# troubling/hummingbird

Hardware: AMD Instinct MI355X
Metric: GiB/s device-resident EC encode+reconstruct, 4+2 @ 1 MiB; % HBM roofline (higher is better)
Workload: dtype u8; 1 GPU; 4+2 Encode + Reconstruct{0,1} of 4096 x 1 MiB objects per GPU, device-resident (BASELINE configs[1]+[2]); k=4, m=2, object_bytes=1048576, objects_per_gpu=4096, global_objects=4096, parallelism=object-partition x1

## Files before the change

hummingbird_amd/csrc/hbec.cpp:

```cpp
#include <hip/hip_runtime.h>

#include <algorithm>
#include <atomic>
#include <condition_variable>
#include <cstdio>
#include <cstdlib>
#include <cstring>
#include <deque>
#include <map>
#include <memory>
#include <mutex>
#include <string>
#include <vector>

#include "../../include/hbec.h"
#include "gf256.h"
#include "internal.h"
#include "kernels.h"
#include "mixed.h"

namespace hbec {

static thread_local std::string t_last_error;

int fail(int code, const std::string& msg) {
    t_last_error = msg;
    return code;
}

int hip_fail(hipError_t e, const char* what) {
    (void)hipGetLastError();
    std::string m = std::string(what) + ": " + hipGetErrorString(e);
    return fail(e == hipErrorOutOfMemory ? HBEC_ERR_NOMEM : HBEC_ERR_DEVICE, m);
}

long long hbec::env_knob(const char* name, long long dflt) {
    const char* e = std::getenv(name);
    return e && *e ? std::atoll(e) : dflt;
}

static std::atomic<int> g_force_stream{0};
static const int g_unaligned_bpc = (int)tune_knob("HBEC_UNALIGNED_BPC", 0);
static const int g_blocks_per_cu_override = (int)tune_knob("HBEC_BLOCKS_PER_CU", 0);
static const int g_grid_cap_env = (int)tune_knob("HBEC_GRID_CAP", 0);
thread_local int t_grid_cap = 0;
void set_thread_grid_cap(int blocks) { t_grid_cap = blocks; }
#define g_grid_cap (t_grid_cap > 0 ? (g_grid_cap_env > 0 ? std::min(t_grid_cap, g_grid_cap_env) : t_grid_cap) : g_grid_cap_env)
static const uint64_t g_chunk_tiles = [] {
    const long long v = tune_knob("HBEC_CHUNK_TILES", 0);
    return (uint64_t)(v > 0 ? v : (1ll << 20));
}();
static std::atomic<uint64_t> g_odd_chunk_override{0};
static uint64_t odd_chunk_tiles() {
    const uint64_t v = g_odd_chunk_override.load(std::memory_order_relaxed);
    return v ? v : g_chunk_tiles;
}
static const uint64_t g_vec_chunk_tiles = [] {
    const long long v = tune_knob("HBEC_VEC_CHUNK_TILES", tune_knob("HBEC_CHUNK_TILES", 0));
    return (uint64_t)(v > 0 ? v : HBEC_VEC_CHUNK_TILES);
}();

struct DeviceInfo {
    int cus = 0;
    std::map<std::pair<int, int>, int> blocks_per_cu;
};

static std::mutex g_dev_mu;
static std::map<int, DeviceInfo> g_devs;

static int bpc_occ_cap(int k, int r) {
    int b = 1;
    if (verify_occupancy(k, r, &b) != hipSuccess) return 1;
    return b;
}

static int current_device(int* dev) {
    hipError_t e = hipGetDevice(dev);
    if (e != hipSuccess) return hip_fail(e, "hipGetDevice");
    return HBEC_OK;
}

static int device_blocks(int dev, int k, int r, int pipe, int force_stream, int* cus, int* per_cu) {
    std::lock_guard<std::mutex> g(g_dev_mu);
    DeviceInfo& d = g_devs[dev];
    if (d.cus == 0) {
        hipDeviceProp_t p;
        hipError_t e = hipGetDeviceProperties(&p, dev);
        if (e != hipSuccess) return hip_fail(e, "hipGetDeviceProperties");
        d.cus = p.multiProcessorCount;
    }
    const int key_k = pipe == 3 ? 3000 : (force_stream ? -k : (pipe == 2 ? 2000 + k : (pipe ? 1000 + k : k)));
    auto it = d.blocks_per_cu.find({key_k, r});
    if (it == d.blocks_per_cu.end()) {
        int b = 0;
        hipError_t e = pipe == 3   ? unaligned_occupancy(r, &b)
                       : pipe == 2 ? packed_occupancy(k, r, &b)
                                   : vec_occupancy(k, r, pipe, force_stream, &b);
        if (e != hipSuccess) return hip_fail(e, "occupancy query");
        if (b < 1) b = 1;
        it = d.blocks_per_cu.emplace(std::make_pair(key_k, r), b).first;
    }
    *cus = d.cus;
    *per_cu = it->second;
    return HBEC_OK;
}

static int cu_count(int dev, int* cus) {
    std::lock_guard<std::mutex> g(g_dev_mu);
    DeviceInfo& d = g_devs[dev];
    if (d.cus == 0) {
        hipDeviceProp_t p;
        hipError_t e = hipGetDeviceProperties(&p, dev);
        if (e != hipSuccess) return hip_fail(e, "hipGetDeviceProperties");
// ... 211 lines not shown
        return apply_wide(rows, cols, coeffs, in, out, n_obj, shard_len, stream);

    for (int r0 = 0; r0 < rows; r0 += kMaxR) {
        const int R = std::min(kMaxR, rows - r0);
        for (int c0 = 0; c0 < cols; c0 += kMaxK) {
            const int K = std::min(kMaxK, cols - c0);
            PassArgs a;
            std::memset(&a, 0, sizeof(a));
            for (int j = 0; j < K; ++j) {
                a.in[j] = static_cast<const uint8_t*>(in[c0 + j].base);
                a.in_stride[j] = in[c0 + j].obj_stride;
            }
            for (int r = 0; r < R; ++r) {
                a.out[r] = static_cast<uint8_t*>(out[r0 + r].base);
                a.out_stride[r] = out[r0 + r].obj_stride;
                for (int j = 0; j < K; ++j) perm_table(coeffs[(size_t)(r0 + r) * cols + c0 + j], a.tab[r][j]);
            }
            a.shard_len = shard_len;
            a.accumulate = c0 > 0 ? 1u : 0u;
            if (vec && is_packed_shape(K, R, shard_len, c0 > 0, force_stream)) {
                int cus = 0, per_cu = 0;
                rc = device_blocks(dev, K, R, 2, 0, &cus, &per_cu);
                if (rc) return rc;
                const uint64_t spo = shard_len / 16;
                const uint64_t te = (uint64_t)packed_tile_elems(K);
                uint64_t max_obj = std::max<uint64_t>(1, ((1ull << 31) - te) / spo);
                max_obj = std::min(max_obj, std::max<uint64_t>(1, g_chunk_tiles * te / spo));
                for (uint64_t o0 = 0; o0 < n_obj; o0 += max_obj) {
                    const uint64_t no = std::min(max_obj, n_obj - o0);
                    PassArgs b = a;
                    for (int j = 0; j < K; ++j) b.in[j] = a.in[j] + o0 * a.in_stride[j];
                    for (int r = 0; r < R; ++r) b.out[r] = a.out[r] + o0 * a.out_stride[r];
                    b.n_obj = no;
                    b.elems_per_obj = (uint32_t)spo;
                    b.n_elems = (uint32_t)(no * spo);
                    b.n_tiles = (uint32_t)((no * spo + te - 1) / te);
                    const uint64_t wpb = (uint64_t)kPipeBlockThreads / 64;
                    const uint64_t want_blocks = (b.n_tiles + wpb - 1) / wpb;
                    const uint64_t cap = (uint64_t)cus * (uint64_t)(g_blocks_per_cu_override > 0
                                                                         ? g_blocks_per_cu_override
                                                                         : per_cu);
                    int grid = (int)std::max<uint64_t>(1, std::min(want_blocks, cap));
                    if (g_grid_cap > 0) grid = std::min(grid, g_grid_cap);
                    hipError_t e = launch_packed(K, R, b, grid, stream);
                    if (e != hipSuccess) return hip_fail(e, "launch gf_apply_packed");
                }
            } else if (vec && !to_rec) {
                int cus = 0, per_cu = 0;
                rc = device_blocks(dev, K, R, is_pipe_shape(K, R, shard_len, force_stream) && c0 == 0, force_stream,
                                   &cus, &per_cu);
                if (rc) return rc;
                const uint64_t tile = (uint64_t)vec_tile_bytes(K, R, shard_len, c0 > 0, force_stream);
                const uint64_t tpo = (shard_len + tile - 1) / tile;
                const uint64_t max_obj = std::max<uint64_t>(1, std::min<uint64_t>((1ull << 31), g_vec_chunk_tiles) / tpo);
                for (uint64_t o0 = 0; o0 < n_obj; o0 += max_obj) {
                    const uint64_t no = std::min(max_obj, n_obj - o0);
                    PassArgs b = a;
                    for (int j = 0; j < K; ++j) b.in[j] = a.in[j] + o0 * a.in_stride[j];
                    for (int r = 0; r < R; ++r) b.out[r] = a.out[r] + o0 * a.out_stride[r];
                    b.n_obj = no;
                    b.tiles_per_obj = (uint32_t)tpo;
                    b.n_tiles = (uint32_t)(no * tpo);
                    const uint64_t wpb = (uint64_t)vec_block_threads(K, R, shard_len, c0 > 0, force_stream) / 64;
                    const uint64_t want_blocks = (b.n_tiles + wpb - 1) / wpb;
                    const uint64_t cap = (uint64_t)cus * (uint64_t)(g_blocks_per_cu_override > 0
                                                                         ? g_blocks_per_cu_override
                                                                         : per_cu);
                    int grid = (int)std::max<uint64_t>(1, std::min(want_blocks, cap));
                    if (g_grid_cap > 0) grid = std::min(grid, g_grid_cap);
                    hipError_t e = launch_vec(K, R, b, grid, stream, force_stream);
                    if (e != hipSuccess) return hip_fail(e, "launch gf_apply_vec");
                }
            } else if (odd_enabled() && cols <= kOddMaxK && pos32_shard(shard_len)) {
                rc = apply_odd(a, K, R, c0 > 0, n_obj, shard_len, dev, stream);
                if (rc) return rc;
            } else {
                int cus = 0, per_cu = 0;
                rc = device_blocks(dev, K, R, 3, 0, &cus, &per_cu);
                if (rc) return rc;
                if (g_unaligned_bpc > 0) per_cu = std::min(per_cu, g_unaligned_bpc);
                const uint64_t tpo = unaligned_tiles_per_obj(shard_len);
                const uint64_t max_obj = std::max<uint64_t>(1, std::min<uint64_t>((1ull << 31), g_chunk_tiles) / tpo);
                for (uint64_t o0 = 0; o0 < n_obj; o0 += max_obj) {
                    const uint64_t no = std::min(max_obj, n_obj - o0);
                    PassArgs b = a;
                    for (int j = 0; j < K; ++j) b.in[j] = a.in[j] + o0 * a.in_stride[j];
                    for (int r = 0; r < R; ++r) b.out[r] = a.out[r] + o0 * a.out_stride[r];
                    b.n_obj = no;
                    b.tiles_per_obj = (uint32_t)tpo;
                    b.n_tiles = (uint32_t)(no * tpo);
                    const uint64_t want_blocks = (b.n_tiles + kBlockThreads / 64 - 1) / (kBlockThreads / 64);
                    int grid = (int)std::max<uint64_t>(1, std::min<uint64_t>(want_blocks, (uint64_t)cus * per_cu));
                    if (g_grid_cap > 0) grid = std::min(grid, g_grid_cap);
                    hipError_t e = launch_unaligned(K, R, b, grid, stream);
                    if (e != hipSuccess) return hip_fail(e, "launch gf_apply_unaligned");
                }
            }
        }
    }
    return HBEC_OK;
}

struct Staging {
    int dev = 0;
    hipStream_t stream = nullptr;
    uint8_t* dbuf = nullptr;
    size_t dcap = 0;
    uint8_t* hbuf = nullptr;
    uint64_t hbuf_dev = 0;
    size_t hcap = 0;
    std::vector<hipEvent_t> ev;
};

static const bool g_percall_mapped = tune_knob("HBEC_PERCALL_DMA", 0) == 0;

static const int g_percall_pieces = (int)std::max(1LL, std::min(16LL, tune_knob("HBEC_PERCALL_PIECES", 2)));

class PercallGate {
  public:
    explicit PercallGate(int limit) : limit_(limit) {}
    void enter() {
        if (limit_ <= 0) return;
        std::unique_lock<std::mutex> lk(mu_);
        if (running_ < limit_ && waiters_.empty()) {
            ++running_;
// ... 363 lines not shown
    const int k = c->k;
    std::vector<MixedRec> recs;
    uint64_t slice[kMaxR + 2] = {};
    std::vector<uint64_t> first;
    uint64_t n_ent = 0;
    for (int r = 1; r <= kMaxR; ++r) {
        slice[r] = n_ent;
        for (MixedPattern& p : pats) {
            if (!p.uses || (int)p.outs.size() != r) continue;
            MixedRec m;
            std::memset(&m, 0, sizeof(m));
            for (int j = 0; j < k; ++j) {
                m.in_base[j] = reinterpret_cast<uint64_t>(views[p.surv[j]].base);
                m.in_stride[j] = views[p.surv[j]].obj_stride;
            }
            for (int q = 0; q < r; ++q) {
                m.out_base[q] = reinterpret_cast<uint64_t>(views[p.outs[q]].base);
                m.out_stride[q] = views[p.outs[q]].obj_stride;
                for (int j = 0; j < k; ++j) perm_table(p.rows[(size_t)q * k + j], m.tab[q][j]);
            }
            p.rec = (uint32_t)recs.size();
            recs.push_back(m);
            first.push_back(n_ent);
            n_ent += p.uses;
        }
    }
    slice[kMaxR + 1] = n_ent;
    if (n_ent == 0) return HBEC_OK;
    std::vector<MixedEnt> ents((size_t)n_ent);
    for (uint64_t o = 0; o < n_objects; ++o) {
        const MixedPattern& p = pats[pattern_of[o]];
        if (p.outs.empty()) continue;
        ents[(size_t)first[p.rec]++] = MixedEnt{(uint32_t)o, p.rec};
    }

    int dev = 0, cus = 0;
    int rc = current_device(&dev);
    if (rc) return rc;
    rc = cu_count(dev, &cus);
    if (rc) return rc;
    const size_t rec_bytes = recs.size() * sizeof(MixedRec), ent_bytes = ents.size() * sizeof(MixedEnt);
    void* d = nullptr;
    rc = scratch_alloc(rec_bytes + ent_bytes, stream, &d);
    if (rc) return rc;
    const MixedRec* d_recs = static_cast<const MixedRec*>(d);
    const MixedEnt* d_ents = reinterpret_cast<const MixedEnt*>(static_cast<const uint8_t*>(d) + rec_bytes);
    hipError_t e = hipMemcpyAsync(d, recs.data(), rec_bytes, hipMemcpyHostToDevice, stream);
    if (e == hipSuccess)
        e = hipMemcpyAsync(const_cast<MixedEnt*>(d_ents), ents.data(), ent_bytes, hipMemcpyHostToDevice, stream);

    const uint64_t tile = (uint64_t)mixed_tile_bytes(k);
    const uint64_t tpo = (shard_len + tile - 1) / tile;
    const uint64_t hook = g_mixed_chunk_override.load(std::memory_order_relaxed);
    const uint64_t max_ent = std::max<uint64_t>(1, std::min<uint64_t>((1ull << 31) - 1, hook ? hook : g_vec_chunk_tiles) / tpo);
    constexpr uint64_t wpb = kBlockThreads / 64;
    for (int r = 1; r <= kMaxR && e == hipSuccess; ++r) {
        for (uint64_t e0 = slice[r]; e0 < slice[r + 1] && e == hipSuccess; e0 += max_ent) {
            const uint64_t ne = std::min(max_ent, slice[r + 1] - e0);
            MixedArgs a;
            a.n_tiles = (uint32_t)(ne * tpo);
            a.tiles_per_obj = (uint32_t)tpo;
            a.shard_len = (uint32_t)shard_len;
            int grid = (int)std::max<uint64_t>(1, std::min<uint64_t>((a.n_tiles + wpb - 1) / wpb, (uint64_t)cus));
            if (g_grid_cap > 0) grid = std::min(grid, g_grid_cap);
            const uint64_t waves = (uint64_t)grid * wpb;
            a.iters = (uint32_t)((a.n_tiles + waves - 1) / waves);
            const uint64_t n_recs = ents[(size_t)(e0 + ne - 1)].rec - ents[(size_t)e0].rec + 1;
            const bool contig = mixed_contiguous(waves, tpo, ne, n_recs);
            a.wave_step = contig ? a.iters : 1u;
            a.iter_step = contig ? 1u : (uint32_t)waves;
            g_mixed_launches.fetch_add(1, std::memory_order_relaxed);
            e = launch_mixed(k, r, a, d_recs, d_ents + e0, grid, stream);
        }
    }
    scratch_free(d, stream);
    if (e != hipSuccess) return hip_fail(e, "launch gf_apply_mixed");
    return HBEC_OK;
}

static int reconstruct_mixed(hbec_codec* c, const hbec_view* views, const uint8_t* patterns, uint32_t n_patterns,
                             const uint32_t* pattern_of, uint64_t n_objects, uint64_t shard_len, bool data_only,
                             hipStream_t stream) {
    if (!c || !views || !patterns || !pattern_of) return fail(HBEC_ERR_INVALID_ARG, "null argument");
    if (n_patterns > 65536) return fail(HBEC_ERR_INVALID_ARG, "more than 65536 patterns");
    if (n_objects && !n_patterns) return fail(HBEC_ERR_INVALID_ARG, "objects but no patterns");
    const int k = c->k, n = c->k + c->m;
    std::vector<MixedPattern> pats(n_patterns);
    std::vector<std::vector<uint8_t>> masks(n_patterns);
    for (uint32_t p = 0; p < n_patterns; ++p) {
        masks[p].assign(patterns + (size_t)p * n, patterns + (size_t)(p + 1) * n);
        int n_present = 0;
        for (auto& v : masks[p]) n_present += (v = v ? 1 : 0);
        if (n_present < k) return fail(HBEC_ERR_TOO_FEW_SHARDS, "too few shards given (pattern " + std::to_string(p) + ")");
    }
    for (uint64_t o = 0; o < n_objects; ++o) {
        if (pattern_of[o] >= n_patterns)
            return fail(HBEC_ERR_INVALID_ARG, "pattern index out of range (object " + std::to_string(o) + ")");
        ++pats[pattern_of[o]].uses;
    }
    bool fast = k <= kMixedMaxK && shard_len % 16 == 0 && pos32_shard(shard_len) && n_objects < (1ull << 32);
    for (uint32_t p = 0; p < n_patterns; ++p) {
        MixedPattern& mp = pats[p];
        if (!mp.uses) continue;
        int rc = decode_rows(c, masks[p], data_only, mp.surv, mp.outs, mp.rows);
        if (rc) return rc;
        if (mp.outs.empty()) continue;
        fast = fast && (int)mp.outs.size() <= kMaxR;
// ... 614 lines not shown
        return HBEC_OK;
    });
}

int hbec_set_odd_chunk_tiles(uint64_t tiles) {
    g_odd_chunk_override.store(tiles, std::memory_order_relaxed);
    return HBEC_OK;
}

int hbec_set_force_stream(int on) {
    return hbec::guarded("hbec_set_force_stream", [&]() -> int {
        g_force_stream.store(on ? 1 : 0);
        return HBEC_OK;
    });
}

int hbec_kernel_info(int k, int r, uint64_t shard_len, int* tile_bytes, int* kind, int* blocks_per_cu) {
    return hbec::guarded("hbec_kernel_info", [&]() -> int {
        if (k < 1 || k > kMaxK || r < 1 || r > kMaxR) return fail(HBEC_ERR_INVALID_ARG, "shape out of range");
        const int fs = g_force_stream.load();
        const bool packed = r <= 3 && is_packed_shape(k, r, shard_len, 0, fs);
        const bool rec = !packed && shard_len % 16 == 0 && rec_route(k, r, shard_len, shard_len % 128 == 0, false);
        const int pipe = packed ? 2 : is_pipe_shape(k, r, shard_len, fs);
        if (tile_bytes)
            *tile_bytes = packed ? packed_tile_elems(k) * 16
                                 : (rec ? (int)odd_rec_tile_span(k, 0, -1) : vec_tile_bytes(k, r, shard_len, 0, fs));
        if (kind) *kind = packed ? 3 : (rec ? 4 : (is_streaming_shape(k, r, fs) ? 2 : (pipe ? 1 : 0)));
        if (blocks_per_cu) {
            int dev = 0, cus = 0;
            int rc = current_device(&dev);
            if (rc) return rc;
            rc = device_blocks(dev, k, r, pipe, packed ? 0 : fs, &cus, blocks_per_cu);
            if (rc) return rc;
            if (rec) *blocks_per_cu = odd_blocks_per_cu(0, k, r, false, true);
            if (g_blocks_per_cu_override > 0) *blocks_per_cu = g_blocks_per_cu_override;
        }
        return HBEC_OK;
    });
}

}

extern "C" int hbec_odd_record_cache(int clear, uint64_t* entries, uint64_t* hits) {
    return hbec::guarded("hbec_odd_record_cache", [&]() -> int {
        ObjRecCache& C = objrec_cache();
        std::lock_guard<std::mutex> lk(C.mu);
        if (clear) {
            hipError_t e = hipDeviceSynchronize();
            if (e != hipSuccess) return hip_fail(e, "hipDeviceSynchronize (record cache)");
            for (auto& x : C.entries) {
                if (x.ev) (void)hipEventDestroy(x.ev);
                if (x.d) (void)hipFree(x.d);
            }
            C.entries.clear();
            C.seen.clear();
            C.bytes = 0;
            C.hits = 0;
        }
        if (entries) *entries = C.entries.size();
        if (hits) *hits = C.hits;
        return HBEC_OK;
    });
}
```

hummingbird_amd/csrc/kernels.h:

```cpp
#pragma once
#include <hip/hip_runtime.h>
#include <stdint.h>

#include "tuning.h"

namespace hbec {

long long env_knob(const char* name, long long dflt);
inline long long tune_knob(const char* name, long long dflt) {
#if HBEC_TUNE
    return env_knob(name, dflt);
#else
    (void)name;
    return dflt;
#endif
}

constexpr int kMaxK = 16;
constexpr uint32_t kOddListWords = 4;
constexpr int kMaxR = 4;
constexpr int kBlockThreads = 256;
constexpr int kPipeBlockThreads = HBEC_PIPE_BLOCK;
constexpr int kPipeBlocksPerCu = HBEC_PIPE_BLOCKS_PER_CU;

constexpr int kVecWavesPerSimd = HBEC_WAVES_PER_SIMD;

struct PassArgs {
    const uint8_t* in[kMaxK];
    uint64_t in_stride[kMaxK];
    uint8_t* out[kMaxR];
    uint64_t out_stride[kMaxR];
    uint32_t tab[kMaxR][kMaxK][5];
    uint64_t n_obj;
    uint64_t shard_len;
    uint32_t tiles_per_obj;
    uint32_t n_tiles;
    uint32_t accumulate;
    uint32_t n_elems;
    uint32_t elems_per_obj;
    uint32_t fuse;
    const uint32_t* list;
};

int is_packed_shape(int k, int r, uint64_t shard_len, int accumulate, int force_stream);
int packed_tile_elems(int k);
hipError_t launch_packed(int k, int r, const PassArgs& a, int grid, hipStream_t stream);
hipError_t packed_occupancy(int k, int r, int* blocks_per_cu);

int vec_tile_bytes(int k, int r, uint64_t shard_len, int accumulate, int force_stream);
int is_streaming_shape(int k, int r, int force_stream);
int is_pipe_shape(int k, int r, uint64_t shard_len, int force_stream);
int vec_block_threads(int k, int r, uint64_t shard_len, int accumulate, int force_stream);
__host__ __device__ constexpr int pipe_u(int k) { return k <= 4 ? (4 / k) : (k <= 8 ? HBEC_PIPE_U_BIG : 1); }

__host__ __device__ constexpr int stripes_u(int k) { return k <= 4 ? pipe_u(k) : 1; }
__host__ __device__ constexpr int verify_u(int k) { return k <= 4 ? 4 : 1; }

hipError_t launch_vec(int k, int r, const PassArgs& a, int grid, hipStream_t stream, int force_stream);
uint32_t unaligned_tiles_per_obj(uint64_t shard_len);
hipError_t launch_unaligned(int k, int r, const PassArgs& a, int grid, hipStream_t stream);
hipError_t unaligned_occupancy(int r, int* blocks_per_cu);
struct URec {
    uint64_t a;
    uint64_t b;
    uint64_t shard_len;
    uint64_t p0;
};
struct UPlanArgs {
    const URec* recs;
    uint32_t n_recs;
    uint32_t accumulate;
    uint32_t in_idx[kMaxK];
    uint32_t out_idx[kMaxR];
    uint32_t in_sel, out_sel;
    uint32_t tab[kMaxR][kMaxK][5];
    uint32_t mirror;
    uint32_t carry;
};
uint32_t unaligned_tile_bytes();
hipError_t launch_verify_unaligned(int k, int r, const PassArgs& a, uint32_t* flags, int grid, hipStream_t stream);
hipError_t launch_unaligned_plan(int k, int r, const UPlanArgs& a, int grid, hipStream_t stream);
constexpr int kOddMaxK = 12;
constexpr uint64_t kPos32MaxShard = (1ull << 31) - (1ull << 16);
__host__ __device__ constexpr bool pos32_shard(uint64_t shard_len) { return shard_len <= kPos32MaxShard; }
bool odd_enabled();
int odd_blocks_per_cu(int mode, int k, int r, bool mirror = false, bool records = false, int xs = -1);
bool odd_supported(int k, int r);
uint64_t urec_tile();
uint64_t urec_tile_for(int k, bool mirror);
uint64_t urec_span(uint64_t shard_len);
uint32_t odd_tile_bytes(int k);
uint32_t odd_plan_tile_bytes();
uint32_t odd_tiles_per_obj(int k, int mode, uint64_t shard_len, bool records, int xs = -1);
uint64_t odd_frame_tiles(uint64_t shard_len, uint64_t tile);
int odd_bp_schedule(int k, int r, int mode, const uint32_t (*tab)[kMaxK][5], bool plan);
uint32_t odd_rec_tile_span(int k, int mode, int xs);
uint32_t odd_waves_per_block(int xs);
uint64_t odd_min_main();
bool odd_uses_records(int k, int r);
uint32_t odd_rec_words(int k, int r, int mode);
hipError_t launch_odd_objrec(int k, int r, int mode, const PassArgs& a, uint32_t* recs, hipStream_t stream);
hipError_t launch_odd_planrec(int k, int r, int mode, const UPlanArgs& p, const URec* orecs, uint32_t n,
                              uint32_t* recs, hipStream_t stream);
hipError_t launch_odd(int k, int r, int mode, const PassArgs& a, uint32_t* flags, const uint32_t* recs, int grid,
// ... 82 lines not shown
```

hummingbird_amd/csrc/kernels.hip:

```cpp
#include <hip/hip_runtime.h>
#include <stdint.h>

#include <cstdlib>
#include <cstring>

#include "gf_device.h"
#include "kernels.h"

namespace hbec {

template <int K, int R, int U>
__device__ __forceinline__ void process_tile(const PassArgs& a, const Tables<K, R>& tb, uint64_t obj,
                                             uint64_t off0, bool full, bool accumulate) {
    u32x4 x[U][K];
    const uint64_t last = a.shard_len - 16u;
#pragma unroll
    for (int u = 0; u < U; ++u) {
        uint64_t off = off0 + (uint64_t)u * 1024u;
        if (!full) off = off < last ? off : last;
#pragma unroll
        for (int j = 0; j < K; ++j) x[u][j] = ld16(a.in[j] + obj * a.in_stride[j] + off);
    }
    u32x4 old[U][R];
    if (accumulate) {
// ... 105 lines not shown
        load_tile<K, R, U>(nxt, a, obj_n, base_n + lane * 16u);
        if (K <= 4) __builtin_amdgcn_s_sleep(HBEC_PIPE_SLEEP);
        if (base + TILE <= a.shard_len)
            compute_store_tile<K, R, U>(cur, a, tb, obj, base + lane * 16u, true);
        else
            compute_store_tile<K, R, U>(cur, a, tb, obj, base + lane * 16u, false);
#pragma unroll
        for (int u = 0; u < U; ++u)
#pragma unroll
            for (int j = 0; j < K; ++j) cur[u][j] = nxt[u][j];
        obj = obj_n;
        base = base_n;
    }
    if (base + TILE <= a.shard_len)
        compute_store_tile<K, R, U>(cur, a, tb, obj, base + lane * 16u, true);
    else
        compute_store_tile<K, R, U>(cur, a, tb, obj, base + lane * 16u, false);
}

template <int K, int R>
struct PipeTile {
    uint64_t in[K];
    uint64_t out[R];
    uint32_t valid;
    uint32_t live;
};

template <int K, int R, int U>
__device__ __forceinline__ void pipe_tile_coords(PipeTile<K, R>& b, const PassArgs& a, uint32_t t, uint32_t tpo) {
    constexpr uint64_t TILE = (uint64_t)U * 1024u;
    const uint32_t obj = t / tpo;
    const uint64_t off = (uint64_t)(t - obj * tpo) * TILE;
#pragma unroll
    for (int j = 0; j < K; ++j) b.in[j] = reinterpret_cast<uint64_t>(a.in[j]) + obj * a.in_stride[j] + off;
#pragma unroll
    for (int r = 0; r < R; ++r) b.out[r] = reinterpret_cast<uint64_t>(a.out[r]) + obj * a.out_stride[r] + off;
    const uint64_t left = a.shard_len - off;
    b.valid = (uint32_t)(left < TILE ? left : TILE);
    b.live = b.valid;
}

template <int K, int R, int U>
__device__ __forceinline__ void pipe2_load(u32x4 (&x)[U][K], const PipeTile<K, R>& b, uint32_t lane) {
    const uint64_t last = (uint64_t)b.valid - 16u;
#pragma unroll
    for (int q = 0; q < U * K; ++q) {
        const int u = HBEC_PIPE_IMAJ ? q % U : q / K, j = HBEC_PIPE_IMAJ ? q / U : q % K;
        uint64_t off = (uint64_t)lane * 16u + (uint64_t)u * 1024u;
        off = off < last ? off : last;
        x[u][j] = HBEC_PIPE_TEMP ? ld16_addr_t(b.in[j] + off) : ld16_addr(b.in[j] + off);
    }
}

template <int K, int R, int U, bool FULL>
__device__ __forceinline__ void pipe2_store_(const u32x4 (&x)[U][K], const PassArgs& a, const Tables<K, R>& tb,
                                             const PipeTile<K, R>& b, uint32_t lane) {
#pragma unroll
    for (int u = 0; u < U; ++u) {
        const uint64_t off = (uint64_t)lane * 16u + (uint64_t)u * 1024u;
        u32x4 acc[R];
#pragma unroll
        for (int r = 0; r < R; ++r) acc[r] = u32x4{0, 0, 0, 0};
        gf_dot<K, R>(acc, x[u], a.tab, tb);
        if (FULL || off < b.live) {
#pragma unroll
            for (int r = 0; r < R; ++r) st16_addr(b.out[r] + off, acc[r]);
        }
    }
}

template <int K, int R, int U>
__device__ __forceinline__ void pipe_tile_at(PipeTile<K, R>& b, const PassArgs& a, uint32_t t, uint32_t n,
                                             uint32_t tpo) {
    pipe_tile_coords<K, R, U>(b, a, t < n ? t : n - 1u, tpo);
    if (t >= n) b.live = 0;
}

template <int K, int R, int U>
__device__ __forceinline__ void pipe2_finish(const u32x4 (&x)[U][K], const PassArgs& a, const Tables<K, R>& tb,
                                             const PipeTile<K, R>& cur, uint32_t lane) {
    if (cur.live >= (uint32_t)U * 1024u)
        pipe2_store_<K, R, U, true>(x, a, tb, cur, lane);
    else
        pipe2_store_<K, R, U, false>(x, a, tb, cur, lane);
}


template <int K, int R>
__global__ __launch_bounds__(kPipeBlockThreads, 1) void gf_apply_vec_pipe2(PassArgs a) {
    constexpr int U = pipe_u(K);
    constexpr uint32_t WPB = kPipeBlockThreads / 64;
    const uint32_t lane = threadIdx.x & 63u;
    const uint32_t nw = gridDim.x * WPB;
    const uint32_t wave0 = __builtin_amdgcn_readfirstlane(xcd_block() * WPB);
    const uint32_t dw = __builtin_amdgcn_readfirstlane(threadIdx.x >> 6);
    const uint32_t wave = wave0 + dw;
    const uint32_t tpo = a.tiles_per_obj;
    const uint32_t n = a.n_tiles;
    if (wave0 >= n) return;
    const Tables<K, R> tb = load_tables<K, R>(a.tab);
    PipeTile<K, R> cur, nxt;
    pipe_tile_at<K, R, U>(cur, a, wave, n, tpo);
    u32x4 x[U][K];
    pipe2_load<K, R, U>(x, cur, lane);
    pipe_tile_at<K, R, U>(nxt, a, wave + nw, n, tpo);
    for (uint32_t b0 = wave0 + nw; b0 < n; b0 += nw) {
        u32x4 y[U][K];
        pipe2_load<K, R, U>(y, nxt, lane);
        if (K <= 4) __builtin_amdgcn_s_sleep(HBEC_PIPE2_SLEEP);
        __builtin_amdgcn_s_barrier();
        PipeTile<K, R> after;
        pipe_tile_at<K, R, U>(after, a, b0 + dw + nw, n, tpo);
        pipe2_finish<K, R, U>(x, a, tb, cur, lane);
#pragma unroll
        for (int u = 0; u < U; ++u)
#pragma unroll
            for (int j = 0; j < K; ++j) x[u][j] = y[u][j];
        cur = nxt;
        nxt = after;
    }
    pipe2_finish<K, R, U>(x, a, tb, cur, lane);
}

template <int K, int U>
__device__ __forceinline__ void packed_load(u32x4 (&x)[U][K], const PassArgs& a, const PackedCoord<U>& c) {
#pragma unroll
    for (int u = 0; u < U; ++u)
#pragma unroll
        for (int j = 0; j < K; ++j) x[u][j] = ld16(a.in[j] + (uint64_t)c.obj[u] * a.in_stride[j] + c.off[u]);
}

template <int K, int R, int U, bool FULL>
__device__ __forceinline__ void packed_store_(const u32x4 (&x)[U][K], const PassArgs& a, const Tables<K, R>& tb,
                                              const PackedCoord<U>& c, uint32_t t, uint32_t lane, uint32_t live) {
#pragma unroll
    for (int u = 0; u < U; ++u) {
        u32x4 acc[R];
#pragma unroll
        for (int r = 0; r < R; ++r) acc[r] = u32x4{0, 0, 0, 0};
        gf_dot<K, R>(acc, x[u], a.tab, tb);
        if (FULL || (t * (uint32_t)U + (uint32_t)u) * 64u + lane < live) {
#pragma unroll
            for (int r = 0; r < R; ++r) st16(a.out[r] + (uint64_t)c.obj[u] * a.out_stride[r] + c.off[u], acc[r]);
        }
    }
}

template <int K, int R, int U>
__device__ __forceinline__ void packed_finish(const u32x4 (&x)[U][K], const PassArgs& a, const Tables<K, R>& tb,
                                              const PackedCoord<U>& c, uint32_t t, uint32_t n, uint32_t lane) {
    const uint32_t live = t < n ? a.n_elems : 0u;
    if (t < n && (t + 1u) * (uint32_t)U * 64u <= a.n_elems)
        packed_store_<K, R, U, true>(x, a, tb, c, t, lane, live);
    else
        packed_store_<K, R, U, false>(x, a, tb, c, t, lane, live);
}


__host__ __device__ constexpr int packed_u(int k) {
    return k > 4 ? HBEC_PACKED_U_BIG : pipe_u(k);
}

template <int K, int R>
__global__ __launch_bounds__(kPipeBlockThreads, 1) void gf_apply_packed(PassArgs a) {
    constexpr int U = packed_u(K);
    constexpr uint32_t WPB = kPipeBlockThreads / 64;
    const uint32_t lane = threadIdx.x & 63u;
    const uint32_t nw = gridDim.x * WPB;
    const uint32_t wave0 = __builtin_amdgcn_readfirstlane(xcd_block() * WPB);
    const uint32_t dw = __builtin_amdgcn_readfirstlane(threadIdx.x >> 6);
    const uint32_t n = a.n_tiles;
    if (wave0 >= n) return;
    const Tables<K, R> tb = load_tables<K, R>(a.tab);
    const uint32_t spo = a.elems_per_obj;
    const double inv = 1.0 / (double)spo;
// ... 391 lines not shown
static uint64_t packed_max_shard(int k) {
    if (k > 4) return HBEC_PACKED_MAX_BIG;
    const uint64_t tile = (uint64_t)pipe_u(k) * 1024u;
    return tile > 2048u ? tile : 2048u;
}

static const bool g_packed_on = tune_knob("HBEC_PACKED", 1) != 0;
static const uint64_t g_packed_max = (uint64_t)std::max(0LL, tune_knob("HBEC_PACKED_MAX_SHARD", 0));

int is_packed_shape(int k, int r, uint64_t shard_len, int accumulate, int force_stream) {
    return (g_packed_on && !force_stream && !accumulate && shard_len >= 16 && shard_len % 16 == 0 &&
            shard_len < (g_packed_max ? g_packed_max : packed_max_shard(k)) &&
            packed_kernel(k, r) != nullptr)
               ? 1
               : 0;
}

hipError_t launch_packed(int k, int r, const PassArgs& a, int grid, hipStream_t stream) {
    const void* fn = packed_kernel(k, r);
    if (!fn) return hipErrorInvalidValue;
    void* args[] = {const_cast<PassArgs*>(&a)};
    return hipLaunchKernel(fn, dim3(grid), dim3(kPipeBlockThreads), args, 0, stream);
}


hipError_t packed_occupancy(int k, int r, int* blocks_per_cu) {
    const void* fn = packed_kernel(k, r);
    if (!fn) return hipErrorInvalidValue;
    hipError_t e = hipOccupancyMaxActiveBlocksPerMultiprocessor(blocks_per_cu, fn, kPipeBlockThreads, 0);
    const int cap = k <= 4 ? HBEC_PACKED_BLOCKS_SMALL : HBEC_PACKED_BLOCKS_BIG;
    if (e == hipSuccess && cap > 0 && *blocks_per_cu > cap) *blocks_per_cu = cap;
    return e;
}

static bool use_pipe(int k, uint64_t shard_len, bool accumulate) {
    return !accumulate && shard_len >= (uint64_t)pipe_u(k) * 1024u;
}

int is_pipe_shape(int k, int r, uint64_t shard_len, int force_stream) {
    return (!is_streaming_shape(k, r, force_stream) && use_pipe(k, shard_len, false)) ? 1 : 0;
}

int vec_tile_bytes(int k, int r, uint64_t shard_len, int accumulate, int force_stream) {
    if (!force_stream && unrolled_kernel(k, r, false))
        return (use_pipe(k, shard_len, accumulate != 0) ? pipe_u(k) : tile_kib(k)) * 1024;
    return 4 * 1024;
}

int vec_block_threads(int k, int r, uint64_t shard_len, int accumulate, int force_stream) {
    return (!is_streaming_shape(k, r, force_stream) && use_pipe(k, shard_len, accumulate != 0)) ? kPipeBlockThreads
                                                                                               : kBlockThreads;
}

hipError_t launch_vec(int k, int r, const PassArgs& a, int grid, hipStream_t stream, int force_stream) {
    const bool pipe = use_pipe(k, a.shard_len, a.accumulate != 0);
    const void* fn = force_stream ? nullptr : unrolled_kernel(k, r, pipe);
    if (fn) {
        void* args[] = {const_cast<PassArgs*>(&a)};
        return hipLaunchKernel(fn, dim3(grid), dim3(pipe ? kPipeBlockThreads : kBlockThreads), args, 0, stream);
    }
    fn = stream_kernel(r);
    if (!fn || k < 1 || k > kMaxK) return hipErrorInvalidValue;
    void* args[] = {const_cast<PassArgs*>(&a), &k};
    return hipLaunchKernel(fn, dim3(grid), dim3(kBlockThreads), args, 0, stream);
}


static const void* unaligned_kernel(int r) {
    switch (r) {
        case 1: return reinterpret_cast<const void*>(&gf_apply_unaligned<1>);
        case 2: return reinterpret_cast<const void*>(&gf_apply_unaligned<2>);
        case 3: return reinterpret_cast<const void*>(&gf_apply_unaligned<3>);
        case 4: return reinterpret_cast<const void*>(&gf_apply_unaligned<4>);
    }
    return nullptr;
}

uint32_t unaligned_tiles_per_obj(uint64_t shard_len) {
    const uint64_t windows = (shard_len + kUnalignedWindow - 1) / kUnalignedWindow;
    return (uint32_t)((windows + kUnalignedU - 1) / kUnalignedU);
}

hipError_t launch_unaligned(int k, int r, const PassArgs& a, int grid, hipStream_t stream) {
    const void* fn = unaligned_kernel(r);
    if (!fn || k < 1 || k > kMaxK) return hipErrorInvalidValue;
    void* args[] = {const_cast<PassArgs*>(&a), &k};
    return hipLaunchKernel(fn, dim3(grid), dim3(kBlockThreads), args, 0, stream);
}

static const void* unaligned_plan_kernel(int r) {
    switch (r) {
        case 1: return reinterpret_cast<const void*>(&gf_apply_unaligned_plan<1>);
        case 2: return reinterpret_cast<const void*>(&gf_apply_unaligned_plan<2>);
        case 3: return reinterpret_cast<const void*>(&gf_apply_unaligned_plan<3>);
        case 4: return reinterpret_cast<const void*>(&gf_apply_unaligned_plan<4>);
    }
    return nullptr;
}

hipError_t launch_verify_unaligned(int k, int r, const PassArgs& a, uint32_t* flags, int grid, hipStream_t stream) {
    const void* fn = nullptr;
    switch (r) {
        case 1: fn = reinterpret_cast<const void*>(&gf_verify_unaligned<1>); break;
        case 2: fn = reinterpret_cast<const void*>(&gf_verify_unaligned<2>); break;
        case 3: fn = reinterpret_cast<const void*>(&gf_verify_unaligned<3>); break;
        case 4: fn = reinterpret_cast<const void*>(&gf_verify_unaligned<4>); break;
    }
    if (!fn || k < 1 || k > kMaxK) return hipErrorInvalidValue;
    void* args[] = {const_cast<PassArgs*>(&a), &k, &flags};
    return hipLaunchKernel(fn, dim3(grid), dim3(kBlockThreads), args, 0, stream);
}

uint32_t unaligned_tile_bytes() { return (uint32_t)kUnalignedU * kUnalignedWindow; }

hipError_t launch_unaligned_plan(int k, int r, const UPlanArgs& a, int grid, hipStream_t stream) {
    const void* fn = unaligned_plan_kernel(r);
    if (!fn || k < 1 || k > kMaxK) return hipErrorInvalidValue;
    void* args[] = {const_cast<UPlanArgs*>(&a), &k};
    return hipLaunchKernel(fn, dim3(grid), dim3(kBlockThreads), args, 0, stream);
}

hipError_t unaligned_occupancy(int r, int* blocks_per_cu) {
    const void* fn = unaligned_kernel(r);
    if (!fn) return hipErrorInvalidValue;
    return hipOccupancyMaxActiveBlocksPerMultiprocessor(blocks_per_cu, fn, kBlockThreads, 0);
}

hipError_t launch_fill(uint8_t* dst, uint64_t n_obj, uint64_t obj_len, uint64_t obj_stride, uint64_t base_seed,
                       uint64_t first, int grid, hipStream_t stream) {
    hipLaunchKernelGGL(fill_splitmix, dim3(grid), dim3(kBlockThreads), 0, stream, dst, n_obj, obj_len, obj_stride,
                       base_seed, first);
    return hipGetLastError();
}

struct PutWords {
    uint32_t n;
    uint32_t w[kPutWordsMax];
};
__global__ __launch_bounds__(kBlockThreads) void put_words(uint32_t* __restrict__ dst, PutWords a) {
    for (uint32_t i = threadIdx.x; i < a.n; i += blockDim.x) dst[i] = a.w[i];
}

hipError_t launch_put_words(void* dst, const void* src, size_t bytes, hipStream_t stream) {
    if (bytes % 4 != 0) return hipErrorInvalidValue;
    const uint32_t* w = static_cast<const uint32_t*>(src);
    uint32_t* d = static_cast<uint32_t*>(dst);
    for (size_t i = 0, n = bytes / 4; i < n; i += kPutWordsMax) {
        PutWords a;
        a.n = (uint32_t)std::min<size_t>(kPutWordsMax, n - i);
        std::memcpy(a.w, w + i, (size_t)a.n * 4);
        hipLaunchKernelGGL(put_words, dim3(1), dim3(kBlockThreads), 0, stream, d + i, a);
        const hipError_t e = hipGetLastError();
        if (e != hipSuccess) return e;
    }
    return hipSuccess;
}

hipError_t vec_occupancy(int k, int r, int pipe, int force_stream, int* blocks_per_cu) {
    const void* fn = force_stream ? nullptr : unrolled_kernel(k, r, pipe != 0);
    const bool is_pipe = fn && pipe;
    if (!fn) fn = stream_kernel(r);
    if (!fn) return hipErrorInvalidValue;
    hipError_t e = hipOccupancyMaxActiveBlocksPerMultiprocessor(blocks_per_cu, fn,
                                                                is_pipe ? kPipeBlockThreads : kBlockThreads, 0);
    if (e == hipSuccess && is_pipe && kPipeBlocksPerCu > 0 && *blocks_per_cu > kPipeBlocksPerCu)
        *blocks_per_cu = kPipeBlocksPerCu;
    return e;
}

}
```

hummingbird_amd/csrc/tuning.h:

```cpp
#pragma once

#ifndef HBEC_TUNE
#define HBEC_TUNE 0
#endif

#ifndef HBEC_PIPE_BLOCK
#define HBEC_PIPE_BLOCK 256
#endif
#ifndef HBEC_PIPE_BLOCKS_PER_CU
#define HBEC_PIPE_BLOCKS_PER_CU 1
#endif
#ifndef HBEC_PIPE_U_BIG
#define HBEC_PIPE_U_BIG 3
#endif
#ifndef HBEC_PIPE_SLEEP
#define HBEC_PIPE_SLEEP 6
#endif
#ifndef HBEC_PIPE2_SLEEP
#define HBEC_PIPE2_SLEEP 8
#endif
#ifndef HBEC_PIPE_IMAJ
#define HBEC_PIPE_IMAJ 0
#endif
#ifndef HBEC_PIPE_TEMP
#define HBEC_PIPE_TEMP 0
#endif
#ifndef HBEC_VEC_CHUNK_TILES
#define HBEC_VEC_CHUNK_TILES 262144
#endif
#ifndef HBEC_PIPE_V2_MAXK
#define HBEC_PIPE_V2_MAXK 4
#endif

#ifndef HBEC_WAVES_PER_SIMD
#define HBEC_WAVES_PER_SIMD 4
#endif
#ifndef HBEC_TILE_SMALL
#define HBEC_TILE_SMALL 4
#endif
#ifndef HBEC_TILE_MID
#define HBEC_TILE_MID 1
#endif
#ifndef HBEC_TILE_BIG
#define HBEC_TILE_BIG 1
#endif

#ifndef HBEC_ALLVGPR_MIN
#define HBEC_ALLVGPR_MIN 16
#endif

#ifndef HBEC_PACKED_U_BIG
#define HBEC_PACKED_U_BIG 1
#endif
#ifndef HBEC_PACKED_MAX_BIG
#define HBEC_PACKED_MAX_BIG 32784
#endif
#ifndef HBEC_PACKED_BLOCKS_SMALL
#define HBEC_PACKED_BLOCKS_SMALL 2
#endif
#ifndef HBEC_PACKED_BLOCKS_BIG
#define HBEC_PACKED_BLOCKS_BIG 1
#endif
#ifndef HBEC_VERIFY_PACKED_U_SMALL
#define HBEC_VERIFY_PACKED_U_SMALL 2
#endif
#ifndef HBEC_VERIFY_PACKED_U_BIG
#define HBEC_VERIFY_PACKED_U_BIG 1
#endif
#ifndef HBEC_VERIFY_PACKED_BLOCKS_SMALL
#define HBEC_VERIFY_PACKED_BLOCKS_SMALL 2
#endif
#ifndef HBEC_VERIFY_PACKED_BLOCKS_BIG
#define HBEC_VERIFY_PACKED_BLOCKS_BIG 2
#endif

#ifndef HBEC_UNALIGNED_U
#define HBEC_UNALIGNED_U 4
#endif

#ifndef HBEC_WIDE_U
#define HBEC_WIDE_U 2
// ... 80 lines not shown
```

Before: 5514 GiB/s.

## Add dynamic atomic tile queue with dedicated claimer wave to pipe2 kernel

Replaces the static grid-stride tile assignment in the pipe2 vector kernel with a dynamic work queue. A dedicated extra wave per block claims tile groups through sharded atomic heads and hands them to the compute waves via a per-block mailbox ring. It also lifts the chunking limit for pipe2 so one launch covers all objects, and splits the static chunk size into its own knob. The aim is better load balance and fewer launches, at the cost of atomic traffic, an extra wave, per-stream persistent queue buffers, and more complex synchronisation.

```diff
diff --git a/hummingbird_amd/csrc/hbec.cpp b/hummingbird_amd/csrc/hbec.cpp
--- a/hummingbird_amd/csrc/hbec.cpp
+++ b/hummingbird_amd/csrc/hbec.cpp
@@ -59,6 +59,71 @@
     const long long v = tune_knob("HBEC_VEC_CHUNK_TILES", tune_knob("HBEC_CHUNK_TILES", 0));
     return (uint64_t)(v > 0 ? v : HBEC_VEC_CHUNK_TILES);
 }();
+static const uint64_t g_vec_static_chunk_tiles = [] {
+    const long long v = tune_knob("HBEC_VEC_STATIC_CHUNK_TILES", tune_knob("HBEC_CHUNK_TILES", 0));
+    return (uint64_t)(v > 0 ? v : HBEC_VEC_STATIC_CHUNK_TILES);
+}();
+#if HBEC_TUNE
+static std::atomic<uint64_t*> g_tune_clk{nullptr};
+extern "C" void hbec_tune_set_clock_buffer(void* p) { g_tune_clk.store(static_cast<uint64_t*>(p)); }
+#endif
+
+namespace {
+struct QueueSlots {
+    std::mutex mu;
+    std::map<std::pair<int, hipStream_t>, uint32_t*> slots;
+};
+constexpr size_t kQueueSlotsMax = 64;
+constexpr size_t kQueueSlotBytes = (size_t)kQueueSlotWords * 4;
+QueueSlots& queue_slots() {
+    static QueueSlots* q = new QueueSlots;
+    return *q;
+}
+}
+
+static int queue_slot(int dev, hipStream_t stream, uint32_t** slot, bool* scratch) {
+    *scratch = false;
+    QueueSlots& Q = queue_slots();
+    {
+        std::lock_guard<std::mutex> g(Q.mu);
+        auto it = Q.slots.find({dev, stream});
+        if (it != Q.slots.end()) {
+            *slot = it->second;
+            return HBEC_OK;
+        }
+        if (stream != hipStreamPerThread && Q.slots.size() < kQueueSlotsMax) {
+            void* d = nullptr;
+            hipError_t e = hipMalloc(&d, kQueueSlotBytes);
+            if (e != hipSuccess) return hip_fail(e, "hipMalloc (tile queue slot)");
+            e = hipMemsetAsync(d, 0, (size_t)kQueueMailWord * 4, stream);
+            if (e != hipSuccess) {
+                (void)hipFree(d);
+                return hip_fail(e, "hipMemsetAsync (tile queue slot)");
+            }
+            *slot = static_cast<uint32_t*>(d);
+            Q.slots.emplace(std::make_pair(dev, stream), *slot);
+            return HBEC_OK;
+        }
+    }
+    void* d = nullptr;
+    int rc = scratch_alloc(kQueueSlotBytes, stream, &d);
+    if (rc) return rc;
+    hipError_t e = hipMemsetAsync(d, 0, (size_t)kQueueMailWord * 4, stream);
+    if (e != hipSuccess) {
+        scratch_free(d, stream);
+        return hip_fail(e, "hipMemsetAsync (tile queue slot)");
+    }
+    *slot = static_cast<uint32_t*>(d);
+    *scratch = true;
+    return HBEC_OK;
+}
+
+static void queue_slots_free() {
+    QueueSlots& Q = queue_slots();
+    std::lock_guard<std::mutex> g(Q.mu);
+    for (auto& x : Q.slots) (void)hipFree(x.second);
+    Q.slots.clear();
+}
 
 struct DeviceInfo {
     int cus = 0;
@@ -376,7 +441,19 @@
                 if (rc) return rc;
                 const uint64_t tile = (uint64_t)vec_tile_bytes(K, R, shard_len, c0 > 0, force_stream);
                 const uint64_t tpo = (shard_len + tile - 1) / tile;
-                const uint64_t max_obj = std::max<uint64_t>(1, std::min<uint64_t>((1ull << 31), g_vec_chunk_tiles) / tpo);
+                const bool queue = is_queue_shape(K, R, shard_len, c0 > 0, force_stream) != 0;
+                const bool pipe2 = is_pipe_shape(K, R, shard_len, force_stream) && c0 == 0 && K <= HBEC_PIPE_V2_MAXK;
+                bool slot_scratch = false;
+                if (queue) {
+                    rc = queue_slot(dev, stream, &a.queue, &slot_scratch);
+                    if (rc) return rc;
+                    per_cu = std::min<int>(per_cu, (int)(kQueueMaxGrid / (uint32_t)std::max(1, cus)));
+                }
+#if HBEC_TUNE
+                a.clk = g_tune_clk.load();
+#endif
+                const uint64_t chunk = pipe2 ? g_vec_chunk_tiles : g_vec_static_chunk_tiles;
+                const uint64_t max_obj = std::max<uint64_t>(1, std::min<uint64_t>((1ull << 31), chunk) / tpo);
                 for (uint64_t o0 = 0; o0 < n_obj; o0 += max_obj) {
                     const uint64_t no = std::min(max_obj, n_obj - o0);
                     PassArgs b = a;
@@ -393,8 +470,12 @@
                     int grid = (int)std::max<uint64_t>(1, std::min(want_blocks, cap));
                     if (g_grid_cap > 0) grid = std::min(grid, g_grid_cap);
                     hipError_t e = launch_vec(K, R, b, grid, stream, force_stream);
-                    if (e != hipSuccess) return hip_fail(e, "launch gf_apply_vec");
+                    if (e != hipSuccess) {
+                        if (slot_scratch) scratch_free(a.queue, stream);
+                        return hip_fail(e, "launch gf_apply_vec");
+                    }
                 }
+                if (slot_scratch) scratch_free(a.queue, stream);
             } else if (odd_enabled() && cols <= kOddMaxK && pos32_shard(shard_len)) {
                 rc = apply_odd(a, K, R, c0 > 0, n_obj, shard_len, dev, stream);
                 if (rc) return rc;
@@ -864,7 +945,7 @@
     const uint64_t tile = (uint64_t)mixed_tile_bytes(k);
     const uint64_t tpo = (shard_len + tile - 1) / tile;
     const uint64_t hook = g_mixed_chunk_override.load(std::memory_order_relaxed);
-    const uint64_t max_ent = std::max<uint64_t>(1, std::min<uint64_t>((1ull << 31) - 1, hook ? hook : g_vec_chunk_tiles) / tpo);
+    const uint64_t max_ent = std::max<uint64_t>(1, std::min<uint64_t>((1ull << 31) - 1, hook ? hook : g_vec_static_chunk_tiles) / tpo);
     constexpr uint64_t wpb = kBlockThreads / 64;
     for (int r = 1; r <= kMaxR && e == hipSuccess; ++r) {
         for (uint64_t e0 = slice[r]; e0 < slice[r + 1] && e == hipSuccess; e0 += max_ent) {
@@ -1585,6 +1666,7 @@
                 if (x.ev) (void)hipEventDestroy(x.ev);
                 if (x.d) (void)hipFree(x.d);
             }
+            queue_slots_free();
             C.entries.clear();
             C.seen.clear();
             C.bytes = 0;
diff --git a/hummingbird_amd/csrc/kernels.h b/hummingbird_amd/csrc/kernels.h
--- a/hummingbird_amd/csrc/kernels.h
+++ b/hummingbird_amd/csrc/kernels.h
@@ -40,7 +40,21 @@
     uint32_t elems_per_obj;
     uint32_t fuse;
     const uint32_t* list;
-};
+    uint32_t* queue;
+#if HBEC_TUNE
+    uint64_t* clk;
+#endif
+};
+
+constexpr uint32_t kQueueHeads = 8;
+constexpr uint32_t kQueueLineWords = 32;
+constexpr uint32_t kQueueDoneWord = kQueueHeads * kQueueLineWords;
+constexpr uint32_t kQueueMailWord = kQueueDoneWord + kQueueLineWords;
+constexpr uint32_t kQueueRing = 8;
+constexpr uint32_t kQueueMaxGrid = 1024;
+constexpr uint32_t kQueueSlotWords = kQueueMailWord + kQueueMaxGrid * kQueueLineWords;
+constexpr uint32_t kQueueEnd = 0xFFFFFFFFu;
+constexpr int kPipe2Threads = HBEC_PIPE_BLOCK + (HBEC_PIPE2_QUEUE ? 64 : 0);
 
 int is_packed_shape(int k, int r, uint64_t shard_len, int accumulate, int force_stream);
 int packed_tile_elems(int k);
@@ -50,6 +64,7 @@
 int vec_tile_bytes(int k, int r, uint64_t shard_len, int accumulate, int force_stream);
 int is_streaming_shape(int k, int r, int force_stream);
 int is_pipe_shape(int k, int r, uint64_t shard_len, int force_stream);
+int is_queue_shape(int k, int r, uint64_t shard_len, int accumulate, int force_stream);
 int vec_block_threads(int k, int r, uint64_t shard_len, int accumulate, int force_stream);
 __host__ __device__ constexpr int pipe_u(int k) { return k <= 4 ? (4 / k) : (k <= 8 ? HBEC_PIPE_U_BIG : 1); }
 
diff --git a/hummingbird_amd/csrc/kernels.hip b/hummingbird_amd/csrc/kernels.hip
--- a/hummingbird_amd/csrc/kernels.hip
+++ b/hummingbird_amd/csrc/kernels.hip
@@ -181,8 +181,8 @@
     }
 }
 
-template <int K, int R, int U, bool FULL>
-__device__ __forceinline__ void pipe2_store_(const u32x4 (&x)[U][K], const PassArgs& a, const Tables<K, R>& tb,
+template <int K, int R, int U, bool FULL, int VMIN>
+__device__ __forceinline__ void pipe2_store_(const u32x4 (&x)[U][K], const PassArgs& a, const Tables<K, R, VMIN>& tb,
                                              const PipeTile<K, R>& b, uint32_t lane) {
 #pragma unroll
     for (int u = 0; u < U; ++u) {
@@ -190,7 +190,7 @@
         u32x4 acc[R];
 #pragma unroll
         for (int r = 0; r < R; ++r) acc[r] = u32x4{0, 0, 0, 0};
-        gf_dot<K, R>(acc, x[u], a.tab, tb);
+        gf_dot<K, R, VMIN>(acc, x[u], a.tab, tb);
         if (FULL || off < b.live) {
 #pragma unroll
             for (int r = 0; r < R; ++r) st16_addr(b.out[r] + off, acc[r]);
@@ -205,18 +205,189 @@
     if (t >= n) b.live = 0;
 }
 
-template <int K, int R, int U>
-__device__ __forceinline__ void pipe2_finish(const u32x4 (&x)[U][K], const PassArgs& a, const Tables<K, R>& tb,
+template <int K, int R, int U, int VMIN>
+__device__ __forceinline__ void pipe2_finish(const u32x4 (&x)[U][K], const PassArgs& a, const Tables<K, R, VMIN>& tb,
                                              const PipeTile<K, R>& cur, uint32_t lane) {
     if (cur.live >= (uint32_t)U * 1024u)
-        pipe2_store_<K, R, U, true>(x, a, tb, cur, lane);
+        pipe2_store_<K, R, U, true, VMIN>(x, a, tb, cur, lane);
     else
-        pipe2_store_<K, R, U, false>(x, a, tb, cur, lane);
-}
-
+        pipe2_store_<K, R, U, false, VMIN>(x, a, tb, cur, lane);
+}
+
+
+#if HBEC_TUNE && HBEC_TUNE_CLOCK
+__device__ __forceinline__ void pipe2_clock(const PassArgs& a, uint32_t which) {
+    if (a.clk && threadIdx.x == 0) a.clk[2u * blockIdx.x + which] = wall_clock64();
+}
+#else
+__device__ __forceinline__ void pipe2_clock(const PassArgs&, uint32_t) {}
+#endif
+
+template <int K, int R, int VMIN>
+__device__ __forceinline__ void pin_scalar_tables(const PassArgs& a) {
+    if constexpr (!Tables<K, R, VMIN>::kAllV) {
+#pragma unroll
+        for (int r = 0; r < R; ++r)
+#pragma unroll
+            for (int j = 0; j < K; ++j)
+                asm volatile("" : : "s"(a.tab[r][j][1]), "s"(a.tab[r][j][3]), "s"(a.tab[r][j][4]));
+    }
+}
+
+#if HBEC_PIPE2_QUEUE
+__device__ __forceinline__ uint32_t queue_fetch(uint32_t* head) {
+    uint32_t v;
+    uint64_t exec_save;
+    const uint32_t one = 1u;
+    asm volatile(
+        "s_mov_b64 %1, exec\n\t"
+        "s_mov_b64 exec, 1\n\t"
+        "global_atomic_add %0, %2, %3, off sc0\n\t"
+        "s_mov_b64 exec, %1"
+        : "=&v"(v), "=&s"(exec_save)
+        : "v"(head), "v"(one)
+        : "memory");
+    return v;
+}
+
+template <int N>
+__device__ __forceinline__ uint32_t queue_result(uint32_t v) {
+    uint32_t c;
+    asm volatile("s_waitcnt vmcnt(%2)\n\tv_readfirstlane_b32 %0, %1" : "=s"(c) : "v"(v), "n"(N) : "memory");
+    return c;
+}
+
+__device__ __forceinline__ uint32_t queue_group(uint32_t h, uint32_t c, uint32_t P, uint32_t nheads) {
+    return nheads == 1u ? c : (c / P) * (kQueueHeads * P) + h * P + c % P;
+}
+
+__device__ __forceinline__ uint32_t queue_entry_load(const uint32_t* mail, uint32_t e) {
+    uint32_t v;
+    const uint32_t* p = mail + e % kQueueRing;
+    asm volatile("s_load_dword %0, %1, 0x0 glc" : "=&s"(v) : "s"(p) : "memory");
+    return v;
+}
+
+__device__ __forceinline__ uint32_t queue_entry_wait(uint32_t v) {
+    uint32_t r;
+    asm volatile("s_waitcnt lgkmcnt(0)\n\ts_mov_b32 %0, %1" : "=s"(r) : "s"(v) : "memory");
+    return r;
+}
+
+template <int D>
+__device__ __forceinline__ void pipe2_claimer(const PassArgs& a, uint32_t n_groups, uint32_t lane) {
+    constexpr uint32_t AHEAD = 1;
+    constexpr uint32_t PRO = 3 + AHEAD;
+    static_assert(kQueueRing >= AHEAD + 3 && kQueueRing <= kQueueLineWords, "hand-off ring");
+    uint32_t* q = a.queue;
+    uint32_t* mail = q + kQueueMailWord + blockIdx.x * kQueueLineWords;
+    const uint32_t nheads = gridDim.x % kQueueHeads == 0u ? kQueueHeads : 1u;
+    const uint32_t P = gridDim.x / nheads;
+    uint32_t h = nheads == 1u ? 0u : blockIdx.x % kQueueHeads;
+    uint32_t tried = 0;
+    uint32_t pend[D];
+    auto fill = [&](const int d0) {
+#pragma unroll
+        for (int j = 0; j < D; ++j) pend[(d0 + j) % D] = queue_fetch(q + h * kQueueLineWords);
+        asm volatile("s_waitcnt vmcnt(0)" ::: "memory");
+    };
+    fill(0);
+    uint32_t e = 0, first_end = 0xFFFFFFFFu;
+    bool more = true;
+    while (more) {
+#pragma unroll
+        for (int d = 0; d < D; ++d) {
+            if (!more) break;
+            uint32_t g = kQueueEnd;
+            while (tried < nheads) {
+                const uint32_t c = queue_result<2 * D - 2>(pend[d]);
+                g = queue_group(h, c, P, nheads);
+                if (g < n_groups) break;
+                g = kQueueEnd;
+                asm volatile("s_waitcnt vmcnt(0)" ::: "memory");
+                if (++tried == nheads) break;
+                h = h + 1u == nheads ? 0u : h + 1u;
+                fill(d);
+            }
+            if (g == kQueueEnd && first_end == 0xFFFFFFFFu) first_end = e;
+            if (lane == 0)
+                __hip_atomic_store(mail + e % kQueueRing, g, __ATOMIC_RELAXED, __HIP_MEMORY_SCOPE_WORKGROUP);
+            if (g != kQueueEnd) pend[d] = queue_fetch(q + h * kQueueLineWords);
+            ++e;
+            if (e >= PRO) {
+                if (e == PRO || tried == nheads)
+                    asm volatile("s_waitcnt vmcnt(0)" ::: "memory");
+                else
+                    asm volatile("s_waitcnt vmcnt(3)" ::: "memory");
+                __builtin_amdgcn_s_barrier();
+                more = (e - PRO) + 1u < first_end;
+            }
+        }
+    }
+    asm volatile("s_waitcnt vmcnt(0)" ::: "memory");
+    uint32_t left = 0;
+    if (lane == 0)
+        left = __hip_atomic_fetch_add(q + kQueueDoneWord, 1u, __ATOMIC_RELAXED, __HIP_MEMORY_SCOPE_AGENT);
+    left = __builtin_amdgcn_readfirstlane(left);
+    if (left + 1u == gridDim.x && lane <= kQueueHeads)
+        __hip_atomic_store(q + lane * kQueueLineWords, 0u, __ATOMIC_RELAXED, __HIP_MEMORY_SCOPE_AGENT);
+}
 
 template <int K, int R>
-__global__ __launch_bounds__(kPipeBlockThreads, 1) void gf_apply_vec_pipe2(PassArgs a) {
+__global__ __launch_bounds__(kPipe2Threads, 1) void gf_apply_vec_pipe2(PassArgs a) {
+    constexpr int U = pipe_u(K);
+    constexpr uint32_t WPB = kPipeBlockThreads / 64;
+    const uint32_t lane = threadIdx.x & 63u;
+    const uint32_t dw = __builtin_amdgcn_readfirstlane(threadIdx.x >> 6);
+    const uint32_t tpo = a.tiles_per_obj;
+    const uint32_t n = a.n_tiles;
+    const uint32_t n_groups = (n + WPB - 1u) / WPB;
+    if (dw == WPB) {
+        pipe2_claimer<HBEC_PIPE2_QDEPTH>(a, n_groups, lane);
+        return;
+    }
+    pipe2_clock(a, 0);
+    const uint32_t* mail = a.queue + kQueueMailWord + blockIdx.x * kQueueLineWords;
+    auto tile_of = [&](uint32_t g) { return g >= n_groups ? n : g * WPB + dw; };
+    constexpr int VMIN = K * R >= 12 ? 1 : HBEC_ALLVGPR_MIN;
+    const Tables<K, R, VMIN> tb = load_tables<K, R, VMIN>(a.tab);
+    pin_scalar_tables<K, R, VMIN>(a);
+    __builtin_amdgcn_s_barrier();
+    asm volatile("" ::: "memory");
+    const uint32_t g0 = queue_entry_wait(queue_entry_load(mail, 0));
+    uint32_t ga = queue_entry_wait(queue_entry_load(mail, 1));
+    uint32_t mv = queue_entry_load(mail, 2);
+    if (g0 == kQueueEnd) return;
+    PipeTile<K, R> cur, nxt;
+    pipe_tile_at<K, R, U>(cur, a, tile_of(g0), n, tpo);
+    u32x4 x[U][K];
+    pipe2_load<K, R, U>(x, cur, lane);
+    pipe_tile_at<K, R, U>(nxt, a, tile_of(ga), n, tpo);
+    for (uint32_t i = 0; ga != kQueueEnd; ++i) {
+        u32x4 y[U][K];
+        pipe2_load<K, R, U>(y, nxt, lane);
+        if (K <= 4) __builtin_amdgcn_s_sleep(HBEC_PIPE2_SLEEP);
+        __builtin_amdgcn_s_barrier();
+        asm volatile("" ::: "memory");
+        const uint32_t gb = queue_entry_wait(mv);
+        mv = queue_entry_load(mail, i + 3u);
+        PipeTile<K, R> after;
+        pipe_tile_at<K, R, U>(after, a, tile_of(gb), n, tpo);
+        pipe2_finish<K, R, U, VMIN>(x, a, tb, cur, lane);
+#pragma unroll
+        for (int u = 0; u < U; ++u)
+#pragma unroll
+            for (int j = 0; j < K; ++j) x[u][j] = y[u][j];
+        cur = nxt;
+        nxt = after;
+        ga = gb;
+    }
+    pipe2_finish<K, R, U, VMIN>(x, a, tb, cur, lane);
+    pipe2_clock(a, 1);
+}
+#else
+template <int K, int R>
+__global__ __launch_bounds__(kPipe2Threads, 1) void gf_apply_vec_pipe2(PassArgs a) {
     constexpr int U = pipe_u(K);
     constexpr uint32_t WPB = kPipeBlockThreads / 64;
     const uint32_t lane = threadIdx.x & 63u;
@@ -227,7 +398,10 @@
     const uint32_t tpo = a.tiles_per_obj;
     const uint32_t n = a.n_tiles;
     if (wave0 >= n) return;
+    pipe2_clock(a, 0);
+    constexpr int VMIN = HBEC_ALLVGPR_MIN;
     const Tables<K, R> tb = load_tables<K, R>(a.tab);
+    pin_scalar_tables<K, R, VMIN>(a);
     PipeTile<K, R> cur, nxt;
     pipe_tile_at<K, R, U>(cur, a, wave, n, tpo);
     u32x4 x[U][K];
@@ -240,7 +414,7 @@
         __builtin_amdgcn_s_barrier();
         PipeTile<K, R> after;
         pipe_tile_at<K, R, U>(after, a, b0 + dw + nw, n, tpo);
-        pipe2_finish<K, R, U>(x, a, tb, cur, lane);
+        pipe2_finish<K, R, U, VMIN>(x, a, tb, cur, lane);
 #pragma unroll
         for (int u = 0; u < U; ++u)
 #pragma unroll
@@ -248,8 +422,10 @@
         cur = nxt;
         nxt = after;
     }
-    pipe2_finish<K, R, U>(x, a, tb, cur, lane);
-}
+    pipe2_finish<K, R, U, VMIN>(x, a, tb, cur, lane);
+    pipe2_clock(a, 1);
+}
+#endif
 
 template <int K, int U>
 __device__ __forceinline__ void packed_load(u32x4 (&x)[U][K], const PassArgs& a, const PackedCoord<U>& c) {
@@ -747,12 +923,22 @@
                                                                                                : kBlockThreads;
 }
 
+static int pipe_threads(int k) { return k <= HBEC_PIPE_V2_MAXK ? kPipe2Threads : kPipeBlockThreads; }
+
+int is_queue_shape(int k, int r, uint64_t shard_len, int accumulate, int force_stream) {
+    return (HBEC_PIPE2_QUEUE && k <= HBEC_PIPE_V2_MAXK && !accumulate && is_pipe_shape(k, r, shard_len, force_stream))
+               ? 1
+               : 0;
+}
+
 hipError_t launch_vec(int k, int r, const PassArgs& a, int grid, hipStream_t stream, int force_stream) {
     const bool pipe = use_pipe(k, a.shard_len, a.accumulate != 0);
     const void* fn = force_stream ? nullptr : unrolled_kernel(k, r, pipe);
     if (fn) {
         void* args[] = {const_cast<PassArgs*>(&a)};
-        return hipLaunchKernel(fn, dim3(grid), dim3(pipe ? kPipeBlockThreads : kBlockThreads), args, 0, stream);
+        if (pipe && HBEC_PIPE2_QUEUE && k <= HBEC_PIPE_V2_MAXK && (!a.queue || grid > (int)kQueueMaxGrid))
+            return hipErrorInvalidValue;
+        return hipLaunchKernel(fn, dim3(grid), dim3(pipe ? pipe_threads(k) : kBlockThreads), args, 0, stream);
     }
     fn = stream_kernel(r);
     if (!fn || k < 1 || k > kMaxK) return hipErrorInvalidValue;
@@ -857,7 +1043,7 @@
     if (!fn) fn = stream_kernel(r);
     if (!fn) return hipErrorInvalidValue;
     hipError_t e = hipOccupancyMaxActiveBlocksPerMultiprocessor(blocks_per_cu, fn,
-                                                                is_pipe ? kPipeBlockThreads : kBlockThreads, 0);
+                                                                is_pipe ? pipe_threads(k) : kBlockThreads, 0);
     if (e == hipSuccess && is_pipe && kPipeBlocksPerCu > 0 && *blocks_per_cu > kPipeBlocksPerCu)
         *blocks_per_cu = kPipeBlocksPerCu;
     return e;
diff --git a/hummingbird_amd/csrc/tuning.h b/hummingbird_amd/csrc/tuning.h
--- a/hummingbird_amd/csrc/tuning.h
+++ b/hummingbird_amd/csrc/tuning.h
@@ -2,6 +2,10 @@
 
 #ifndef HBEC_TUNE
 #define HBEC_TUNE 0
+#endif
+
+#ifndef HBEC_TUNE_CLOCK
+#define HBEC_TUNE_CLOCK 1
 #endif
 
 #ifndef HBEC_PIPE_BLOCK
@@ -25,8 +29,17 @@
 #ifndef HBEC_PIPE_TEMP
 #define HBEC_PIPE_TEMP 0
 #endif
+#ifndef HBEC_PIPE2_QUEUE
+#define HBEC_PIPE2_QUEUE 1
+#endif
+#ifndef HBEC_PIPE2_QDEPTH
+#define HBEC_PIPE2_QDEPTH 2
+#endif
+#ifndef HBEC_VEC_STATIC_CHUNK_TILES
+#define HBEC_VEC_STATIC_CHUNK_TILES 262144
+#endif
 #ifndef HBEC_VEC_CHUNK_TILES
-#define HBEC_VEC_CHUNK_TILES 262144
+#define HBEC_VEC_CHUNK_TILES 2147483648
 #endif
 #ifndef HBEC_PIPE_V2_MAXK
 #define HBEC_PIPE_V2_MAXK 4
```

After: 5564 GiB/s, median of 6. Within noise of the previous version (+0.9%).
